# ulysses4ever/SparseMatrixVBCs.jl

Measured on AMD Instinct MI355X. Metric: 1DVBC SpMV effective GB/s (and GFLOP/s) vs HBM roofline, 1/2/4/8 GPU, higher is better.
Workload: dtype f64; 1 GPU; FE-2D-5pt-dof2-10Mx10M-1e8nnz-w2 (SuiteSparse-like mesh operator); op=mul!(y, B', x) -- transposed 1DVBC (multiply_1DVBC.jl:85-180), m=9999392, n=9999392, stripes=4999696, row_blocks=49979072, nnz=99958144, W=8, index_bytes=4, nrhs=1, launch=hipGraph of K products, layout_bytes=826106369, cache=matrix > MALL: every product streams the layout from HBM, parallelism=single GPU

## Files before the change

include/vbc.h:

```cpp
#ifndef VBC_H
#define VBC_H

#ifndef VBC_API
#define VBC_API __attribute__((visibility("default")))
#endif

#include <stddef.h>
#include <stdint.h>

#define VBC_VERSION 30200
#define VBC_INFO_SIZE 152

#ifdef __cplusplus
extern "C" {
#endif

typedef enum vbc_status {
    VBC_OK = 0,
    VBC_DIM_MISMATCH = 1,
    VBC_INVALID_ARG = 2,
    VBC_HIP_ERROR = 3,
    VBC_RCCL_ERROR = 4,
    VBC_UNSUPPORTED_DTYPE = 5,
    VBC_ASSERTION = 6
} vbc_status;

// ... 105 lines not shown
    int32_t device;
    int32_t bins_t, bins_f;
    int64_t device_bytes;
    int64_t bytes_t;
    int64_t bytes_f;
    int32_t bins_m;
    int32_t slot_bins;
    int64_t bytes_m;
    int32_t sweep_bins;
    int32_t planar_bins;
    int32_t planar_run;
    int32_t planar_split;
    int32_t planar_pair;
    int32_t fwd_run;
    int32_t planar_mask;
} vbc_info;

VBC_API int vbc_get_info(const vbc_handle *h, vbc_info *info);

VBC_API int vbc_last_error(char *buf, size_t n);

VBC_API int vbc_version(void);

#ifdef __cplusplus
}
#endif
#endif
```

include/vbc_host.h:

```cpp
#ifndef VBC_HOST_H
#define VBC_HOST_H

#ifndef VBC_API
#define VBC_API __attribute__((visibility("default")))
#endif

#include <stdint.h>

#ifdef __cplusplus
extern "C" {
#endif

VBC_API int vbcx_partition_equi(int64_t n, int64_t w, int64_t *spl, int64_t *L);

VBC_API int vbcx_partition_strict(int64_t m, int64_t n, const int64_t *colptr, const int64_t *rowval,
                          int64_t W, int64_t *spl, int64_t *L);

VBC_API int vbcx_partition_overlap(int64_t m, int64_t n, const int64_t *colptr, const int64_t *rowval,
                           double rho, int64_t W, int64_t *spl, int64_t *L);

VBC_API int vbcx_partition_dynamic(int64_t m, int64_t n, const int64_t *colptr, const int64_t *rowval,
                           int64_t W, double c_stripe, double c_col, double c_pin, double c_row,
                           double c_cell, int64_t *spl, int64_t *L);

// ... 9 lines not shown
                     const int64_t *spl, int64_t *pos, int64_t *ofs);
VBC_API int vbcx_1dvbc_fill(int64_t m, int64_t n, int64_t W, const int64_t *colptr, const int64_t *rowval,
                    const void *nzval, int dtype, int64_t L, const int64_t *spl, const int64_t *pos,
                    const int64_t *ofs, int64_t *idx, void *val, int64_t pad);

VBC_API int vbcx_vbc_count(int64_t m, int64_t n, const int64_t *colptr, const int64_t *rowval, int64_t K,
                   const int64_t *pspl, int64_t L, const int64_t *spl, int64_t *pos, int64_t *ofs);
VBC_API int vbcx_vbc_fill(int64_t m, int64_t n, int64_t U, int64_t W, const int64_t *colptr,
                  const int64_t *rowval, const void *nzval, int dtype, int64_t K,
                  const int64_t *pspl, int64_t L, const int64_t *spl, const int64_t *pos,
                  const int64_t *ofs, int64_t *idx, void *val, int64_t pad);

VBC_API int vbcx_transpose_pattern(int64_t m, int64_t n, const int64_t *colptr, const int64_t *rowval,
                           int64_t *rowptr, int64_t *colval);

#ifdef __cplusplus
}
#endif
#endif
```

sparsematrixvbcs.jl_amd/_lib.py:

```python
import ctypes as C
import os
from pathlib import Path

import numpy as np

PKG_DIR = Path(__file__).resolve().parent
LIB_PATH = Path(os.environ.get("VBC_LIBRARY", PKG_DIR / "libvbc.so"))

VBC_OK, VBC_DIM_MISMATCH, VBC_INVALID_ARG, VBC_HIP_ERROR, VBC_RCCL_ERROR, VBC_UNSUPPORTED_DTYPE, \
    VBC_ASSERTION = range(7)
VBC_F64, VBC_F32, VBC_I64, VBC_I32, VBC_BOOL = range(5)
VBC_MEM_DEVICE, VBC_MEM_HOST = 0, 1
VBC_CREATE_TRANSPOSED, VBC_CREATE_FORWARD, VBC_CREATE_MULTI, VBC_CREATE_SERIAL = 0x1, 0x2, 0x4, 0x8
VBC_CREATE_MULTI_FORWARD = 0x10
VBC_VERSION_MAJOR = 3
VBC_INFO_SIZE = 152
VBC_MUL_REFERENCE_QUIRKS = 0x1
VBC_MAT_ROWMAJOR = 0x2
VBC_SPLIT_STRIPES, VBC_SPLIT_ROWS, VBC_SPLIT_AUTO = 0, 1, 2

ABI_SYMBOLS = (
    "vbc1d_create", "vbc2d_create", "vbc_csc_create", "vbc_destroy", "vbc_mul", "vbc_mul_mat",
    "vbc1d_create_ex", "vbc2d_create_ex", "vbc_csc_create_ex", "vbc_mul_ex", "vbc_mul_mat_ex",
    "vbc_get_info", "vbc_last_error", "vbc_version",
    "vbc1d_create_sharded", "vbc2d_create_sharded", "vbc_sharded_mul", "vbc_sharded_mul_ex", "vbc_sharded_destroy",
    "vbc_sharded_count", "vbc_sharded_shard", "vbc_sharded_split", "vbc_sharded_xspan",
    "vbcx_partition_equi", "vbcx_partition_strict", "vbcx_partition_overlap",
    "vbcx_partition_dynamic", "vbcx_partition_dynamic_table", "vbcx_partition_block", "vbcx_1dvbc_count", "vbcx_1dvbc_fill", "vbcx_vbc_count",
    "vbcx_vbc_fill", "vbcx_transpose_pattern",
)


class DimensionMismatch(ValueError):
    """Julia's DimensionMismatch (multiply_1DVBC.jl:44-45,139-140)."""


class ArgumentError(ValueError):
    """Julia's ArgumentError (SparseMatrixVBCs.jl:45-50,72-79)."""


class HIPError(RuntimeError):
    pass


# ... 4 lines not shown
class vbc_types(C.Structure):
    _fields_ = [("val_dtype", C.c_int32), ("index_bits", C.c_int32), ("compute_dtype", C.c_int32),
                ("reserved", C.c_int32)]


class vbc_info(C.Structure):
    _fields_ = [("m", C.c_int64), ("n", C.c_int64), ("L", C.c_int64), ("K", C.c_int64),
                ("nblocks", C.c_int64), ("nrows", C.c_int64), ("nval", C.c_int64),
                ("nnz_hint", C.c_int64), ("dtype", C.c_int32), ("device", C.c_int32),
                ("bins_t", C.c_int32), ("bins_f", C.c_int32), ("device_bytes", C.c_int64),
                ("bytes_t", C.c_int64), ("bytes_f", C.c_int64), ("bins_m", C.c_int32),
                ("slot_bins", C.c_int32), ("bytes_m", C.c_int64),
                ("sweep_bins", C.c_int32), ("planar_bins", C.c_int32),
                ("planar_run", C.c_int32), ("planar_split", C.c_int32),
                ("planar_pair", C.c_int32), ("fwd_run", C.c_int32),
                ("planar_mask", C.c_int32)]


_lib = None


def lib():
    global _lib
    if _lib is None:
        if not LIB_PATH.exists():
            raise ImportError(f"libvbc.so not found at {LIB_PATH}; build it with `make -C {PKG_DIR}` "
                              "or __graft_entry__.build()")
        try:
            import torch
        except ImportError:
            pass
# ... 27 lines not shown
        L.vbc_mul_mat.argtypes = [P, INT, I64, P, I64, I64, P, I64, I64, D, D, INT, P, U]
        L.vbc_mul_mat_ex.argtypes = [P, INT, I64, P, INT, I64, I64, P, INT, I64, I64, D, D, INT, P, U]
        L.vbc_get_info.argtypes = [P, C.POINTER(vbc_info)]
        L.vbc_last_error.argtypes = [C.c_char_p, C.c_size_t]
        L.vbcx_partition_equi.argtypes = [I64, I64, P, P]
        L.vbcx_partition_strict.argtypes = [I64, I64, P, P, I64, P, P]
        L.vbcx_partition_overlap.argtypes = [I64, I64, P, P, D, I64, P, P]
        L.vbcx_partition_dynamic.argtypes = [I64, I64, P, P, I64, D, D, D, D, D, P, P]
        L.vbcx_partition_dynamic_table.argtypes = [I64, I64, P, P, I64, P, P, P, P]
        L.vbcx_partition_block.argtypes = [I64, I64, P, P, P, I64, I64, P, I64, P, P, P, P]
        L.vbcx_1dvbc_count.argtypes = [I64, I64, P, P, I64, P, P, P]
        L.vbcx_1dvbc_fill.argtypes = [I64, I64, I64, P, P, P, INT, I64, P, P, P, P, P, I64]
        L.vbcx_vbc_count.argtypes = [I64, I64, P, P, I64, P, I64, P, P, P]
        L.vbcx_vbc_fill.argtypes = [I64, I64, I64, I64, P, P, P, INT, I64, P, I64, P, P, P, P, P, I64]
        L.vbcx_transpose_pattern.argtypes = [I64, I64, P, P, P, P]
        _lib = L
    return _lib


def last_error():
    buf = C.create_string_buffer(1024)
    lib().vbc_last_error(buf, 1024)
    return buf.value.decode(errors="replace")


def check(status, what=""):
    if status == VBC_OK:
        return
    msg = f"{what}: {last_error()}" if what else last_error()
    if status == VBC_DIM_MISMATCH:
# ... 37 lines not shown
```

sparsematrixvbcs.jl_amd/csrc/vbc_device.hip:

```cpp
#include <hip/hip_runtime.h>

#include <algorithm>
#include <array>
#include <cstdarg>
#include <cstring>
#include <cmath>
#include <map>
#include <string>
#include <type_traits>
#include <unordered_map>
#include <vector>

#include "vbc_handle.h"
#include "vbc_planar.h"

namespace vbc {

static thread_local std::string g_err;

void set_error(const char *fmt, ...)
{
    char buf[1024];
    va_list ap;
    va_start(ap, fmt);
// ... 407 lines not shown
    int64_t nr = (int64_t)std::llround(share);
    const double quantum = share / std::max(1, planar ? h->occ_p : h->occ_s[kind]);
    if (!planar && h->range_bytes > 0 && share >= 2 * quantum) {
        const double bytes = (double)rows * RPI * (w * esz + 4);
        if (bytes / share < (double)h->range_bytes) nr = (int64_t)std::llround(share / 2);
    }
    const int wps = (pair && h->planar_wps_pair > 0) ? h->planar_wps_pair : h->planar_wps;
    if (planar && split == 1 && wps > 0) nr = std::min<int64_t>(nr, std::max<int64_t>(1, std::llround(quantum * wps)));
    nr = std::max<int64_t>(1, std::min<int64_t>(nr, nch));
    const int64_t qi = (int64_t)quantum;
    if (split == 1 && qi >= 1 && nr < (int64_t)std::llround(share) && nr > qi) nr = nr / qi * qi;
    if (split > 1) nr = nch;
    bool affine = true;
    for (size_t q = 1; q < out.size() && affine; q++)
        affine = (int64_t)out[q] == (int64_t)out[0] + (int64_t)q * (out[1] - out[0]);
    std::vector<int32_t> rrow{0}, rchunk{0};
    int64_t acc = 0;
    for (int64_t c = 0; c < nch; c++) {
        acc += cr[c];
        const bool full = split > 1 || (!affine && (int64_t)(c + 2 - rchunk.back()) * RPI > kSlotOutEntries);
        if (c + 1 < nch && (full || ((int64_t)rrow.size() < nr && acc * nr >= (int64_t)rrow.size() * rows))) {
            rrow.push_back((int32_t)acc);
            rchunk.push_back((int32_t)(c + 1));
        }
    }
    rrow.push_back((int32_t)rows);
    nr = (int64_t)rchunk.size();
    if (layout_knob("VBC_VERBOSE"))
        fprintf(stderr, "[vbc] slot bin kind %d w %d planar %d pair %d run %d split %d chunks %lld rows %lld ranges %lld "
                "(target share %.0f)\n", kind, w, (int)planar, (int)pair, run, split, (long long)nch, (long long)rows,
                (long long)nr, share);
    ps = PendingSlot{};
    SlotBin &b = ps.b;
    b.kind = kind;
    b.wkey = w <= 8 ? w : 0;
    b.w = w;
    b.wst = wsrc;
    b.rpi = RPI;
    b.range0 = range0;
    b.nranges = (int32_t)nr;
    b.nseg = (int32_t)nstripes;
    b.ks = ks;
    b.fused = (planar && kind == 0 && split > 1 && h->small_split > 1 && wsrc <= 8 && ((h->fuse_w >> wsrc) & 1)) ? 1 : 0;
    b.u = h->slot_u;
    b.diag = h->diag;
    b.xcd = (planar && split == 1) ? h->xcd_p : 0;
    b.nowonly = h->slot_wonly ? 0 : 1;
    b.spl = slot_spl(h, kind, w);
    b.planar = planar ? 1 : 0;
    b.run = run;
    b.split = split;
    b.pair = pair ? 1 : 0;
    b.mask = (mask && planar && split == 1 && (!pair || h->planar_mask_pair)) ? 1 : 0;
    b.holes = holes ? 1 : 0;
    if (holes && (split == 1 || pair)) return fail(VBC_INVALID_ARG, "internal: runs with holes need the split product");
    if (planar && split > 1) {
        const double rows_per_wave = (double)rows / (double)std::max<int64_t>(nch, 1) / split;
        const int u0 = (9 / w) / run * run;
        const double step_rows = (double)std::min(8 * run, std::max(run, u0));
        b.deep = h->split_pipe >= 0 ? h->split_pipe : (b.fused && rows_per_wave > h->split_deep * step_rows ? 2 : 0);
        if (b.deep == 2 && h->split_nt_bytes > 0 && (double)h->nval * h->esz > (double)h->split_nt_bytes) b.deep = 3;
    }
    b.out_affine = 1;
    b.out_base = out.empty() ? 0 : out[0];
    b.out_stride = out.size() > 1 ? out[1] - out[0] : 0;
    for (size_t q = 1; q < out.size() && b.out_affine; q++)
        b.out_affine = (int64_t)out[q] == (int64_t)out[0] + (int64_t)q * b.out_stride;
    if (ablation_knob("VBC_NO_AFFINE")) b.out_affine = 0;
// ... 49 lines not shown
                        key[e] = kPad | last;
                    }
                    blk[4 * sl + 0] = v[0][0];
                    blk[4 * sl + 1] = v[0][1];
                    blk[4 * sl + 2] = v[0][2];
                    blk[4 * sl + 3] = v[1][2];
                    blk[128 + 2 * sl + 0] = v[1][0];
                    blk[128 + 2 * sl + 1] = v[1][1];
                    blk[192 + sl] = v[2][2];
                    blk[224 + 2 * sl + 0] = v[2][0];
                    blk[224 + 2 * sl + 1] = v[2][1];
                }
            }
        }
    }
    for (int64_t c = 0; c < (pair ? 0 : nch); c++) {
        for (int32_t qr = 0; qr < cr[c]; qr++, row++) {
            const uint32_t last = qr + run == cr[c] ? kLast : 0u;
            if (b.mask) {
                uint32_t nl = 0;
                for (int sl = 0; sl < RPI; sl++) {
                    const int64_t seg = c * RPI + sl;
                    if (seg < nseg && sbeg[seg] + qr < sbeg[seg + 1]) {
                        if (nl != (uint32_t)sl) return fail(VBC_INVALID_ARG, "masked planar chunk: live lanes not a prefix");
                        nl++;
                    }
                }
                ar.at<uint32_t>(ps.o_nlive)[row] = nl;
            }
            for (int sl = 0; sl < RPI; sl++) {
                const int64_t seg = c * RPI + sl, e = row * RPI + sl;
// ... 1994 lines not shown
    if (const char *e = layout_knob("VBC_SLOTS_PAD")) h->slots_pad = atof(e);
    if (const char *e = layout_knob("VBC_SLOTS_SORT")) h->slots_sort = atoi(e);
    if (const char *e = tuning_knob("VBC_SLOT_NARROW")) h->slot_narrow = atoi(e) != 0;
    if (const char *e = layout_knob("VBC_XCD")) h->xcd = atoi(e) != 0;
    if (const char *e = layout_knob("VBC_XCD_P")) h->xcd_p = atoi(e) != 0;
    if (const char *e = layout_knob("VBC_SLOT_KEYS16")) h->slot_keys16 = atoi(e);
    if (const char *e = layout_knob("VBC_SLOT_DEDUP")) h->slot_dedup = atoi(e) != 0;
    if (const char *e = layout_knob("VBC_SWEEP")) h->sweep_mode = atoi(e) == 0 ? 0 : atoi(e) == 1 ? 1 : -1;
    h->sweep_tile = (h->esz == 8 ? 4 : 2) * kSweepTileBytes;
    h->sweep_pack = h->esz == 8;
    if (const char *e = layout_knob("VBC_FORK")) h->fork = atoi(e) != 0;
    if (const char *e = tuning_knob("VBC_FORK_SIDE_KB")) h->fork_side_bytes = atof(e) * 1024.0;
    if (const char *e = layout_knob("VBC_SWEEP_PACK")) h->sweep_pack = atoi(e) != 0;
    if (const char *e = layout_knob("VBC_SWEEP_TILE")) h->sweep_tile = atoi(e) >= 32 ? 4 * kSweepTileBytes : atoi(e) >= 16 ? 2 * kSweepTileBytes : kSweepTileBytes;
    if (const char *e = layout_knob("VBC_SLOT_STAGE")) h->slot_stage = (atoi(e) == 4 || atoi(e) == 8) ? atoi(e) : 0;
    if (const char *e = layout_knob("VBC_SLOT_PLANAR")) h->slot_planar = atoi(e) == 0 ? 0 : atoi(e) == 1 ? 1 : -1;
    if (const char *e = layout_knob("VBC_SLOT_RUNS")) h->slot_runs = atoi(e) != 0;
    if (const char *e = layout_knob("VBC_PLANAR_PAIR")) h->planar_pair = atoi(e) == 0 ? 0 : atoi(e) == 2 ? 2 : 1;
    if (const char *e = layout_knob("VBC_PLANAR_MASK")) h->planar_mask = atoi(e) != 0;
    if (const char *e = layout_knob("VBC_PLANAR_MASK_PAIR")) h->planar_mask_pair = atoi(e) != 0;
    if (const char *e = layout_knob("VBC_MASK_WINDOW")) h->mask_window = std::max(1, std::min(64, atoi(e)));
    if (const char *e = layout_knob("VBC_PLANAR_SPLIT")) {
        const int v = atoi(e);
        h->planar_split = v == 0 ? 0 : (v == 2 || v == 4 || v == 8) ? v : -1;
    }
    if (flags & VBC_CREATE_SERIAL) {
        h->planar_split = 0;
        if (h->slots_mode < 0) h->slots_mode = 1;
    }
    h->occ_p = std::max(1, std::min(occupancy_planar(h->esz), 8));
    h->target_ranges_l = prop.multiProcessorCount * std::max(1, std::min(occupancy_lanes(h->esz), 8)) * kWavesPerBlock;
    if (const char *e = layout_knob("VBC_PLANAR_LANES")) h->planar_lanes = atoi(e) == 0 ? 0 : atoi(e) == 1 ? 1 : -1;
    if (const char *e = layout_knob("VBC_TARGET_RANGES_L")) h->target_ranges_l = std::max(1, atoi(e));
    if (const char *e = tuning_knob("VBC_LANES_DEEP")) h->lanes_deep = atoi(e) != 0;
    if (const char *e = tuning_knob("VBC_LANES_RDIV")) h->lanes_rdiv = std::max(1, atoi(e));
    if (const char *e = layout_knob("VBC_LANES_PAIR")) h->lanes_pair = atoi(e) != 0;
    if (const char *e = tuning_knob("VBC_SPLIT_KC")) h->split_kc = atoi(e) != 0;
    if (const char *e = tuning_knob("VBC_SPLIT_ROWS")) h->split_rows = std::max(1, atoi(e));
    if (const char *e = layout_knob("VBC_SMALL_FUSE")) h->small_fuse = atoi(e);
    if (const char *e = layout_knob("VBC_SIDE_FUSE")) h->side_fuse = atoi(e) < 0 ? -1 : atoi(e) != 0;
    if (const char *e = layout_knob("VBC_COLSPLIT")) h->colsplit = atoi(e) != 0;
    if (const char *e = tuning_knob("VBC_FUSE_PMAX")) h->fuse_pmax = atoi(e) >= 8 ? 8 : atoi(e) >= 4 ? 4 : 2;
    if (const char *e = tuning_knob("VBC_COLSPLIT_W")) h->colsplit_w = std::max(0, atoi(e));
// ... 381 lines not shown
        for (const SlotBin &b : h->lt.pbins)
            if (b.ks > 1) info->planar_mask |= 64;
    info->fwd_run = 1;
    if (h->has_f)
        for (const auto &l : h->lf)
            for (const auto &b : l.pbins) {
                info->fwd_run = std::max<int32_t>(info->fwd_run, b.lanes ? b.wkey : b.run);
                if (b.mask && !b.lanes) info->planar_mask |= 2;
                if (b.split > 1) info->planar_mask |= 8;
                if (b.lanes) info->planar_mask |= 16;
                if (b.dot) info->planar_mask |= 2048;
            }
    if (h->has_ft)
        for (const SlotBin &b : h->lft.pbins)
            if (b.split > 1) info->planar_mask |= 8;
    info->bytes_m = h->has_m ? h->bytes_m : h->bytes_mf;
    return VBC_OK;
}

static int check_mul(const vbc_handle *h, int trans, int64_t nx, int64_t ny, bool mat = false)
{
    if (!h) return fail(VBC_INVALID_ARG, "NULL handle");
    const int64_t want_x = trans ? h->m : h->n, want_y = trans ? h->n : h->m;
    if (nx != want_x || ny != want_y) return fail(VBC_DIM_MISMATCH, "DimensionMismatch");
    if (trans && !h->has_t && !(mat && h->has_m))
        return fail(VBC_INVALID_ARG, mat ? "handle built without VBC_CREATE_TRANSPOSED or VBC_CREATE_MULTI"
                                         : "handle built without VBC_CREATE_TRANSPOSED");
    if (!trans && !h->has_f && !(mat && h->has_mf))
        return fail(VBC_INVALID_ARG, mat ? "handle built without VBC_CREATE_FORWARD or VBC_CREATE_MULTI_FORWARD"
                                         : "handle built without VBC_CREATE_FORWARD");
// ... 357 lines not shown
```

sparsematrixvbcs.jl_amd/csrc/vbc_handle.h:

```cpp
#pragma once
#include <hip/hip_runtime.h>

#include <cstdint>
#include <mutex>
#include <vector>

#include "vbc_internal.h"
#include "vbc_kernels.h"
#include "vbc_panel.h"
#include "vbc_tiles.h"

namespace vbc {

#define VBC_HIP(call)                                                                             \
    do {                                                                                          \
        hipError_t e_ = (call);                                                                   \
        if (e_ != hipSuccess) {                                                                   \
            set_error("%s failed: %s", #call, hipGetErrorString(e_));                             \
            return VBC_HIP_ERROR;                                                                 \
        }                                                                                         \
    } while (0)

struct Launch {
    std::vector<Bin> bins;
// ... 95 lines not shown
    int slots_mode = -1;
    double slots_pad = 1.10;
    int slot_narrow = 1;
    int slots_sort = 1;
    int xcd = 1;
    int64_t range_bytes = 192 << 10;
    int xcd_p = 1;
    int occ_s[2] = {4, 4};
    int64_t slot_rows_padded = 0, slot_rows_real = 0;
    int64_t slot_rows_padded_last = 0;
    int slot_u = 0;
    bool slot_dedup = true;
    int slot_keys16 = 1;
    int fork = 1;
    int slot_stage = -1;
    int slot_planar = -1;
    int slot_runs = 1;
    int planar_pair = 1;
    int planar_mask = 1;
    int planar_mask_pair = 1;
    int mask_window = 2;
    int planar_split = -1;
    int target_ranges_p = 4096;
    int target_ranges_l = 4096;
    int slot_wonly = 1;
    int split_kc = 0;
    int small_split = 0;
    uint32_t fuse_w = 0;
    int small_fuse = 1;
    int side_fuse = -1;
// ... 54 lines not shown
```

sparsematrixvbcs.jl_amd/csrc/vbc_host.cpp:

```cpp
#include <algorithm>
#include <cmath>
#include <cstdlib>
#include <cstring>
#include <limits>
#include <thread>
#include <vector>

#include "vbc_host.h"
#include "vbc_internal.h"

using vbc::fail;

namespace {

int host_threads()
{
    if (const char *e = std::getenv("VBC_HOST_THREADS")) return std::max(1, std::atoi(e));
    const unsigned hc = std::thread::hardware_concurrency();
    return (int)std::max(1u, std::min(hc ? hc : 1u, 16u));
}

template <typename F>
int parallel_ranges(int64_t n, int64_t work, F f)
{
// ... 417 lines not shown
int vbcx_transpose_pattern(int64_t m, int64_t n, const int64_t *colptr, const int64_t *rowval,
                           int64_t *rowptr, int64_t *colval)
{
    if (int st = check_csc(m, n, colptr, rowval)) return st;
    std::fill(rowptr, rowptr + m + 1, 0);
    for (int64_t p = 0; p < colptr[n] - 1; p++) rowptr[rowval[p]]++;
    rowptr[0] = 1;
    for (int64_t i = 0; i < m; i++) rowptr[i + 1] += rowptr[i];
    std::vector<int64_t> next(rowptr, rowptr + m);
    for (int64_t j = 0; j < n; j++)
        for (int64_t p = colptr[j] - 1; p < colptr[j + 1] - 1; p++)
            colval[(next[rowval[p] - 1]++) - 1] = j + 1;
    return VBC_OK;
}

}
```

sparsematrixvbcs.jl_amd/csrc/vbc_internal.h:

```cpp
#pragma once
#include <cstdarg>
#include <cstdint>
#include <cstdio>
#include <cstdlib>

#include "vbc.h"

namespace vbc {

void set_error(const char *fmt, ...) __attribute__((format(printf, 1, 2)));

inline int fail(int status, const char *what)
{
    set_error("%s", what);
    return status;
}

inline const char *layout_knob(const char *name) { return std::getenv(name); }
#ifdef VBC_ABLATION
#define VBC_ABL(expr) (expr)
inline const char *ablation_knob(const char *name) { return std::getenv(name); }
inline const char *tuning_knob(const char *name) { return std::getenv(name); }
#else
#define VBC_ABL(expr) 0
inline const char *ablation_knob(const char *) { return nullptr; }
inline const char *tuning_knob(const char *) { return nullptr; }
#endif

inline int elem_size(int dtype)
{
    switch (dtype) {
    case VBC_F64: case VBC_I64: return 8;
    case VBC_F32: case VBC_I32: return 4;
    case VBC_BOOL: return 1;
    default: return 0;
    }
}

template <typename To>
void host_convert(const void *src, int dt, int64_t n, int64_t inc, To *dst)
{
    const char *p = static_cast<const char *>(src);
// ... 35 lines not shown
```

sparsematrixvbcs.jl_amd/csrc/vbc_kernels.h:

```cpp
#pragma once
#include <hip/hip_runtime.h>

#include <cstdint>

#include "vbc_internal.h"

namespace vbc {

constexpr int kBlockThreads = 256;
constexpr int kWavesPerBlock = kBlockThreads / 64;
constexpr int kTileKDefault = 8;
constexpr int kPipeDefault = 2;
constexpr uint32_t kHead = 0x80000000u;

template <typename T>
using gptr = __attribute__((address_space(1))) T *;
template <typename T>
__device__ __forceinline__ gptr<T> G(T *p) { return (gptr<T>)p; }
template <typename T>
__device__ __forceinline__ gptr<const T> G(const T *p) { return (gptr<const T>)p; }

template <typename V>
__device__ __forceinline__ void st_y(gptr<V> p, V v, bool nt)
{
// ... 58 lines not shown
    const uint32_t *base;
    const uint32_t *kdoff;
    const void *val;
    const int32_t *out;
    const int32_t *rrow;
    const int32_t *rchunk;
    const uint32_t *nlive;
    int32_t lanes;
    int32_t ntiles;
    int32_t deep;
    int32_t nowonly;
    const int32_t *trow;
    const int32_t *tseg;
    const int16_t *lseg;
    int32_t dot;
    int32_t pad_dot;
};

constexpr uint32_t kHoleIdx = (1u << 27) - 1;
constexpr int kHoleShift = 27;

constexpr int kSplitParts = 16;
struct SplitPart {
    int32_t w, run, chunk0, nseg, out_affine, out_base, out_stride, wst, holes, ks;
    const int32_t *rrow;
    const uint32_t *key;
    const void *val;
    const int32_t *out;
};
struct SplitMulti {
    int32_t nparts, nchunks, pad0, pad1;
// ... 779 lines not shown
```

sparsematrixvbcs.jl_amd/csrc/vbc_slots.h:

```cpp
#pragma once
#include "vbc_kernels.h"

namespace vbc {

template <typename T, int V>
__device__ __forceinline__ T slot_reduce(const T (&v)[V], int lane, int sub, int LPR)
{
    T s = T(0);
#pragma unroll
    for (int e = 0; e < V; e++) s += v[e];
    for (int d = 1; d < LPR; d <<= 1) {
        const T t = __shfl(s, (lane + d) & 63, 64);
        if (sub + d < LPR) s += t;
    }
    return s;
}

template <typename T, int KIND, int W_, int U, bool FASTE, int DIAG = 0, int NB = 0, bool KC = false>
__device__ __forceinline__ void run_slots(const SlotBin &b, int r, int lane, const T *__restrict__ x,
                                          T *__restrict__ y, T alpha, T beta, bool rd, char *lds_wave, int *lds_out)
{
    constexpr bool kGeneric = (W_ == 0);
    constexpr int V = kGeneric ? 1 : vec_elems(sizeof(T), W_);
    const int w = kGeneric ? b.w : W_;
    const int LPR = kGeneric ? b.w : W_ / V;
    const int RPI = b.rpi;
    const int slot = lane / LPR, sub = lane - slot * LPR;
    const bool active = slot < RPI;
    const int R0 = G(b.rrow)[r], R1 = G(b.rrow)[r + 1];
    if (R0 >= R1) return;
    int c = G(b.rchunk)[r];
    const int lslot = active ? slot : 0, lsub = active ? sub : 0;
    const gptr<const T> val = G(static_cast<const T *>(b.val));
    const gptr<const uint32_t> key = G(b.key);
    const gptr<const T> xg = G(x);
    constexpr int XV = KIND == 0 ? 1 : V;

    typedef __attribute__((address_space(4))) const uint32_t *cptr;
    const cptr bases = (cptr)b.base;
    const cptr doffs = (cptr)b.kdoff;
    auto load = [&](int R, uint32_t (&kk)[U], uint32_t (&bs)[U], T (&v)[U][V]) {
#pragma unroll
        for (int u = 0; u < U; u++) {
            const int Rc = min(R + u, R1 - 1);
            const size_t p = (size_t)Rc * RPI + lslot;
            if constexpr (KC) {
// ... 7 lines not shown
        }
    };
    constexpr uint32_t kPad16 = 0xFFFF8000u;
    auto gather = [&](const uint32_t (&kk)[U], const uint32_t (&bs)[U], T (&xv)[U][XV]) {
#pragma unroll
        for (int u = 0; u < U; u++) {
            const uint32_t gi = KC ? (bs[u] & kSlotIdx) + (kk[u] == kPad16 ? 0u : kk[u]) : kk[u] & kSlotIdx;
#pragma unroll
            for (int e = 0; e < XV; e++) xv[u][e] = DIAG == 2 ? T(1) : xg[gi + (KIND == 0 ? 0 : lsub * V + e)];
        }
    };
    T acc[V], dump[V];
#pragma unroll
    for (int e = 0; e < V; e++) acc[e] = dump[e] = T(0);
    int nbuf = 0, cfirst = c;
    const int c0 = c;
    if constexpr (!FASTE) {
        if (!b.out_affine) {
            const int n = min(kSlotOutEntries, b.nseg - c0 * RPI);
            for (int i = lane; i < n; i += 64) lds_out[i] = G(b.out)[c0 * RPI + i];
        }
    }

    auto write_out = [&]() {
        const int64_t segs = min((int64_t)nbuf * RPI, (int64_t)b.nseg - (int64_t)cfirst * RPI);
        const int64_t bytes = segs * (KIND == 0 ? w : 1) * (int64_t)sizeof(T);
        char *dst = reinterpret_cast<char *>(y + b.out_base + (int64_t)cfirst * RPI * b.out_stride);
        if ((reinterpret_cast<uintptr_t>(dst) & 15) == 0) {
            typedef uint32_t u4 __attribute__((ext_vector_type(4)));
            for (int64_t off = (int64_t)lane * 16; off < bytes; off += 1024) {
// ... 17 lines not shown
        if constexpr (NB > 0) {
            if constexpr (KIND == 0) {
                typedef T vt __attribute__((ext_vector_type(V)));
                vt t;
#pragma unroll
                for (int e = 0; e < V; e++) t[e] = alpha * acc[e];
                *reinterpret_cast<vt *>(lds_wave + ((size_t)nbuf * 64 + lane) * V * sizeof(T)) = t;
            } else {
                const T s = slot_reduce<T, V>(acc, lane, sub, LPR);
                if (sub == 0 && active) reinterpret_cast<T *>(lds_wave)[(size_t)nbuf * RPI + slot] = alpha * s;
            }
#pragma unroll
            for (int e = 0; e < V; e++) acc[e] = T(0);
            if (nbuf == 0) cfirst = c;
            c++;
            if (++nbuf == NB) write_out();
            return;
        }
        if constexpr (KIND == 0) {
            if (ok) {
                const int o = (FASTE || b.out_affine) ? b.out_base + seg * b.out_stride : lds_out[(c - c0) * RPI + slot];
                gptr<T> yo = DIAG == 4 ? G(y) + ((size_t)r * 64 + lane) * V : G(y) + o + sub * V;
                const int lim = b.wst - sub * V;
                T q[V];
#pragma unroll
                for (int e = 0; e < V; e++) {
                    q[e] = alpha * acc[e];
                    if (!FASTE && rd && e < lim) q[e] = fmadd(beta, yo[e], q[e]);
                }
                if constexpr (DIAG == 1) {
#pragma unroll
// ... 12 lines not shown
                }
            }
        } else {
            const T s = slot_reduce<T, V>(acc, lane, sub, LPR);
            if (ok && sub == 0) {
                const int o = (FASTE || b.out_affine) ? b.out_base + seg * b.out_stride : lds_out[(c - c0) * RPI + slot];
                gptr<T> yo = G(y) + o;
                T q = alpha * s;
                if (!FASTE && rd) q = fmadd(beta, *yo, q);
                *yo = q;
            }
        }
#pragma unroll
        for (int e = 0; e < V; e++) acc[e] = T(0);
        c++;
    };
    int R1v;
    asm volatile("v_mov_b32 %0, %1" : "=v"(R1v) : "s"(R1));
    auto compute = [&](int R, const uint32_t (&kk)[U], const uint32_t (&bs)[U], const T (&v)[U][V],
                       const T (&xv)[U][XV]) {
#pragma unroll
        for (int u = 0; u < U; u++) {
            const bool live = R + u < R1v;
            const bool pad = KC ? kk[u] == kPad16 : (kk[u] & kPad) != 0;
#pragma unroll
            for (int e = 0; e < V; e++) {
                const T xe = pad ? T(0) : xv[u][KIND == 0 ? 0 : e];
                const T nv = fmadd(v[u][e], xe, acc[e]);
                acc[e] = live ? nv : acc[e];
            }
// ... 21 lines not shown
#pragma unroll
        for (int e = 0; e < V; e++) G(y)[(size_t)(blockIdx.x * kBlockThreads + threadIdx.x) * V + e] = dump[e];
    }
}

template <typename T, int W_, int SPL, int U, bool FASTE, int NB, bool KC>
__device__ __forceinline__ void run_slots_narrow(const SlotBin &b, int r, int lane, const T *__restrict__ x,
                                                 T *__restrict__ y, T alpha, T beta, bool rd, char *lds_wave,
                                                 int *lds_out)
{
    constexpr int NV = SPL * W_;
    const int RPI = b.rpi;
    const int R0 = G(b.rrow)[r], R1 = G(b.rrow)[r + 1];
    if (R0 >= R1) return;
    int c = G(b.rchunk)[r];
    const gptr<const T> val = G(static_cast<const T *>(b.val));
    const gptr<const T> xg = G(x);
    typedef __attribute__((address_space(4))) const uint32_t *cptr;
    const cptr bases = (cptr)b.base;
    const cptr doffs = (cptr)b.kdoff;
    typedef T vt __attribute__((ext_vector_type(NV)));
    auto load = [&](int R, uint32_t (&kk)[U][SPL], uint32_t (&bs)[U], T (&v)[U][NV]) {
#pragma unroll
        for (int u = 0; u < U; u++) {
            const int Rc = min(R + u, R1 - 1);
            const size_t p = (size_t)Rc * RPI + (size_t)lane * SPL;
            if constexpr (KC) {
                typedef int16_t hv __attribute__((ext_vector_type(SPL)));
                const hv d = *(gptr<const hv>)((gptr<const int16_t>)b.key + (size_t)doffs[Rc] + (size_t)lane * SPL);
#pragma unroll
// ... 13 lines not shown
    };
    constexpr uint32_t kPad16 = 0xFFFF8000u;
    auto is_pad = [&](uint32_t k) { return KC ? k == kPad16 : (k & kPad) != 0; };
    auto gather = [&](const uint32_t (&kk)[U][SPL], const uint32_t (&bs)[U], T (&xv)[U][SPL]) {
#pragma unroll
        for (int u = 0; u < U; u++)
#pragma unroll
            for (int k = 0; k < SPL; k++) {
                const uint32_t gi = KC ? (bs[u] & kSlotIdx) + (kk[u][k] == kPad16 ? 0u : kk[u][k]) : kk[u][k] & kSlotIdx;
                xv[u][k] = xg[gi];
            }
    };
    T acc[NV];
#pragma unroll
    for (int e = 0; e < NV; e++) acc[e] = T(0);
    int nbuf = 0, cfirst = c;
    const int c0 = c;
    if constexpr (!FASTE) {
        if (!b.out_affine) {
            const int n = min(kSlotOutEntries, b.nseg - c0 * RPI);
            for (int i = lane; i < n; i += 64) lds_out[i] = G(b.out)[c0 * RPI + i];
        }
    }
    auto write_out = [&]() {
        const int64_t segs = min((int64_t)nbuf * RPI, (int64_t)b.nseg - (int64_t)cfirst * RPI);
        const int64_t bytes = segs * W_ * (int64_t)sizeof(T);
        char *dst = reinterpret_cast<char *>(y + b.out_base + (int64_t)cfirst * RPI * b.out_stride);
        if ((reinterpret_cast<uintptr_t>(dst) & 15) == 0) {
            typedef uint32_t u4 __attribute__((ext_vector_type(4)));
            for (int64_t off = (int64_t)lane * 16; off < bytes; off += 1024) {
                if (off + 16 <= bytes) {
// ... 34 lines not shown
#pragma unroll
                        for (int e = 0; e < W_; e++) {
                            if (e >= lim) break;
                            T q = alpha * acc[k * W_ + e];
                            if (!FASTE && rd) q = fmadd(beta, G(y)[o + e], q);
                            G(y)[o + e] = q;
                        }
                    }
                }
            }
        }
#pragma unroll
        for (int e = 0; e < NV; e++) acc[e] = T(0);
        c++;
        if constexpr (NB > 0) {
            if (++nbuf == NB) write_out();
        }
    };
    int R1v;
    asm volatile("v_mov_b32 %0, %1" : "=v"(R1v) : "s"(R1));
    auto compute = [&](int R, const uint32_t (&kk)[U][SPL], const uint32_t (&bs)[U], const T (&v)[U][NV],
                       const T (&xv)[U][SPL]) {
#pragma unroll
        for (int u = 0; u < U; u++) {
            const bool live = R + u < R1v;
#pragma unroll
            for (int k = 0; k < SPL; k++) {
                const T xe = is_pad(kk[u][k]) ? T(0) : xv[u][k];
#pragma unroll
                for (int e = 0; e < W_; e++) {
                    const T nv = fmadd(v[u][k * W_ + e], xe, acc[k * W_ + e]);
// ... 81 lines not shown
```

Measured before the change: 7245 GB/s.

## Interleave slot-bin chunk ranges into sweeping pieces to align x gather locality

Adds a host planner that samples column-offset deltas in transposed slot bins and, when a few dominant far offsets exist, reorders chunks so each wave range processes strided pieces of P chunks and all ranges sweep the matrix together. Concurrent waves then touch nearby x regions, which is meant to improve cache reuse of the x gather. The kernels gain a piece counter that jumps chunk indices after each burst. It also adds equal-sized range counting by default and exposes the plan in the info struct. The risks are more irregular output write bursts and a heuristic that may pick poor plans or none at all.

```diff
diff --git a/include/vbc.h b/include/vbc.h
--- a/include/vbc.h
+++ b/include/vbc.h
@@ -8,8 +8,8 @@
 #include <stddef.h>
 #include <stdint.h>
 
-#define VBC_VERSION 30200
-#define VBC_INFO_SIZE 152
+#define VBC_VERSION 30300
+#define VBC_INFO_SIZE 160
 
 #ifdef __cplusplus
 extern "C" {
@@ -145,6 +145,9 @@
     int32_t planar_pair;
     int32_t fwd_run;
     int32_t planar_mask;
+    int32_t slot_sweep_p;
+    int32_t slot_sweep_s;
+    int32_t slot_sweep_r;
 } vbc_info;
 
 VBC_API int vbc_get_info(const vbc_handle *h, vbc_info *info);
diff --git a/include/vbc_host.h b/include/vbc_host.h
--- a/include/vbc_host.h
+++ b/include/vbc_host.h
@@ -47,6 +47,9 @@
 VBC_API int vbcx_transpose_pattern(int64_t m, int64_t n, const int64_t *colptr, const int64_t *rowval,
                            int64_t *rowptr, int64_t *colval);
 
+VBC_API int vbcx_slot_sweep_plan(int64_t chunks, int64_t slots, int nb, int ndelta, const double *delta,
+                                 const double *weight, int force_p, int force_s, int64_t *plan);
+
 #ifdef __cplusplus
 }
 #endif
diff --git a/sparsematrixvbcs.jl_amd/_lib.py b/sparsematrixvbcs.jl_amd/_lib.py
--- a/sparsematrixvbcs.jl_amd/_lib.py
+++ b/sparsematrixvbcs.jl_amd/_lib.py
@@ -14,7 +14,7 @@
 VBC_CREATE_TRANSPOSED, VBC_CREATE_FORWARD, VBC_CREATE_MULTI, VBC_CREATE_SERIAL = 0x1, 0x2, 0x4, 0x8
 VBC_CREATE_MULTI_FORWARD = 0x10
 VBC_VERSION_MAJOR = 3
-VBC_INFO_SIZE = 152
+VBC_INFO_SIZE = 160
 VBC_MUL_REFERENCE_QUIRKS = 0x1
 VBC_MAT_ROWMAJOR = 0x2
 VBC_SPLIT_STRIPES, VBC_SPLIT_ROWS, VBC_SPLIT_AUTO = 0, 1, 2
@@ -27,7 +27,7 @@
     "vbc_sharded_count", "vbc_sharded_shard", "vbc_sharded_split", "vbc_sharded_xspan",
     "vbcx_partition_equi", "vbcx_partition_strict", "vbcx_partition_overlap",
     "vbcx_partition_dynamic", "vbcx_partition_dynamic_table", "vbcx_partition_block", "vbcx_1dvbc_count", "vbcx_1dvbc_fill", "vbcx_vbc_count",
-    "vbcx_vbc_fill", "vbcx_transpose_pattern",
+    "vbcx_vbc_fill", "vbcx_transpose_pattern", "vbcx_slot_sweep_plan",
 )
 
 
@@ -62,7 +62,8 @@
                 ("sweep_bins", C.c_int32), ("planar_bins", C.c_int32),
                 ("planar_run", C.c_int32), ("planar_split", C.c_int32),
                 ("planar_pair", C.c_int32), ("fwd_run", C.c_int32),
-                ("planar_mask", C.c_int32)]
+                ("planar_mask", C.c_int32), ("slot_sweep_p", C.c_int32),
+                ("slot_sweep_s", C.c_int32), ("slot_sweep_r", C.c_int32)]
 
 
 _lib = None
@@ -120,6 +121,7 @@
         L.vbcx_vbc_count.argtypes = [I64, I64, P, P, I64, P, I64, P, P, P]
         L.vbcx_vbc_fill.argtypes = [I64, I64, I64, I64, P, P, P, INT, I64, P, I64, P, P, P, P, P, I64]
         L.vbcx_transpose_pattern.argtypes = [I64, I64, P, P, P, P]
+        L.vbcx_slot_sweep_plan.argtypes = [I64, I64, INT, INT, P, P, INT, INT, P]
         _lib = L
     return _lib
 
diff --git a/sparsematrixvbcs.jl_amd/csrc/vbc_device.hip b/sparsematrixvbcs.jl_amd/csrc/vbc_device.hip
--- a/sparsematrixvbcs.jl_amd/csrc/vbc_device.hip
+++ b/sparsematrixvbcs.jl_amd/csrc/vbc_device.hip
@@ -445,9 +445,67 @@
     bool affine = true;
     for (size_t q = 1; q < out.size() && affine; q++)
         affine = (int64_t)out[q] == (int64_t)out[0] + (int64_t)q * (out[1] - out[0]);
+    SweepPlan sweep;
+    {
+        const int V0 = w <= 8 ? vec_elems(esz, w) : 1;
+        const bool full0 = slot_spl(h, kind, w) > 1 || (RPI * (w / V0) == 64 && V0 * esz <= 16);
+        const int64_t ostride = out.size() > 1 ? (int64_t)out[1] - out[0] : 0;
+        const bool eligible = h->slot_sweep != 0 && kind == 0 && !planar && split == 1 && ks == 1 && order.empty() &&
+                              !mask && affine && !ablation_knob("VBC_NO_AFFINE") && full0 && wsrc == w &&
+                              (nseg <= 1 || ostride == w) && nch >= 2;
+        if (eligible && h->slot_sweep == 2) {
+            sweep = plan_slot_sweep(nch, nr, 8, 0, nullptr, nullptr, h->slot_sweep_p, h->slot_sweep_s);
+        } else if (eligible && nch >= nr) {
+            std::unordered_map<int64_t, int64_t> hist;
+            std::vector<int64_t> all;
+            const int64_t step = std::max<int64_t>(1, nseg / 65536);
+            for (int64_t q = 0; q < nseg; q += step)
+                for (int64_t t = sbeg[q]; t < sbeg[q + 1]; t++) {
+                    const int64_t d = (int64_t)(ents[pstart[q] + (t - sbeg[q])].key & kSlotIdx) - (int64_t)out[q];
+                    all.push_back(d >= 0 ? d / w : -((-d + w - 1) / w));
+                }
+            if (!all.empty()) {
+                std::nth_element(all.begin(), all.begin() + all.size() / 2, all.end());
+                const int64_t med = all[all.size() / 2];
+                int64_t far = 0;
+                for (int64_t d : all)
+                    if (std::llabs(d - med) > (int64_t)8 * RPI) {
+                        hist[d - med]++;
+                        far++;
+                    }
+                std::vector<double> dl, wt;
+                int64_t dom = 0;
+                for (const auto &kv : hist)
+                    if (kv.second * 10 >= far) {
+                        dl.push_back((double)kv.first / RPI);
+                        wt.push_back((double)kv.second);
+                        dom += kv.second;
+                    }
+                if (far * 20 >= (int64_t)all.size() && dom * 5 >= far * 4)
+                    sweep = plan_slot_sweep(nch, nr, 8, (int)dl.size(), dl.data(), wt.data(), 0, 0);
+            }
+        }
+    }
+    if (sweep.P == 0 && h->slot_equal && !planar && split == 1 && affine && nch > nr) nr = equal_range_count(nch, nr);
+    std::vector<int64_t> lorder;
     std::vector<int32_t> rrow{0}, rchunk{0};
     int64_t acc = 0;
-    for (int64_t c = 0; c < nch; c++) {
+    if (sweep.P > 0) {
+        const int64_t P = sweep.P, pieces = (nch + P - 1) / P;
+        lorder.reserve(nch);
+        for (int64_t r = 0; r < sweep.R; r++) {
+            for (int64_t p = r; p < pieces; p += sweep.R)
+                for (int64_t c = p * P; c < std::min(nch, (p + 1) * P); c++) {
+                    lorder.push_back(c);
+                    acc += cr[c];
+                }
+            if (r + 1 < sweep.R) {
+                rrow.push_back((int32_t)acc);
+                rchunk.push_back((int32_t)((r + 1) * P));
+            }
+        }
+    }
+    for (int64_t c = 0; c < (sweep.P > 0 ? 0 : nch); c++) {
         acc += cr[c];
         const bool full = split > 1 || (!affine && (int64_t)(c + 2 - rchunk.back()) * RPI > kSlotOutEntries);
         if (c + 1 < nch && (full || ((int64_t)rrow.size() < nr && acc * nr >= (int64_t)rrow.size() * rows))) {
@@ -459,8 +517,8 @@
     nr = (int64_t)rchunk.size();
     if (layout_knob("VBC_VERBOSE"))
         fprintf(stderr, "[vbc] slot bin kind %d w %d planar %d pair %d run %d split %d chunks %lld rows %lld ranges %lld "
-                "(target share %.0f)\n", kind, w, (int)planar, (int)pair, run, split, (long long)nch, (long long)rows,
-                (long long)nr, share);
+                "(target share %.0f) pieces of %d chunks, %lld sweeps (lag %.3f)\n", kind, w, (int)planar, (int)pair, run,
+                split, (long long)nch, (long long)rows, (long long)nr, share, (int)sweep.P, (long long)sweep.S, sweep.lag);
     ps = PendingSlot{};
     SlotBin &b = ps.b;
     b.kind = kind;
@@ -483,6 +541,7 @@
     b.split = split;
     b.pair = pair ? 1 : 0;
     b.mask = (mask && planar && split == 1 && (!pair || h->planar_mask_pair)) ? 1 : 0;
+    b.piece = sweep.P;
     b.holes = holes ? 1 : 0;
     if (holes && (split == 1 || pair)) return fail(VBC_INVALID_ARG, "internal: runs with holes need the split product");
     if (planar && split > 1) {
@@ -562,7 +621,8 @@
             }
         }
     }
-    for (int64_t c = 0; c < (pair ? 0 : nch); c++) {
+    for (int64_t lc = 0; lc < (pair ? 0 : nch); lc++) {
+        const int64_t c = lorder.empty() ? lc : lorder[lc];
         for (int32_t qr = 0; qr < cr[c]; qr++, row++) {
             const uint32_t last = qr + run == cr[c] ? kLast : 0u;
             if (b.mask) {
@@ -2587,6 +2647,17 @@
     if (const char *e = layout_knob("VBC_SWEEP_PACK")) h->sweep_pack = atoi(e) != 0;
     if (const char *e = layout_knob("VBC_SWEEP_TILE")) h->sweep_tile = atoi(e) >= 32 ? 4 * kSweepTileBytes : atoi(e) >= 16 ? 2 * kSweepTileBytes : kSweepTileBytes;
     if (const char *e = layout_knob("VBC_SLOT_STAGE")) h->slot_stage = (atoi(e) == 4 || atoi(e) == 8) ? atoi(e) : 0;
+    if (const char *e = layout_knob("VBC_SLOT_SWEEP")) {
+        if (e[0] == 'p' || e[0] == 'P') {
+            h->slot_sweep = 2;
+            h->slot_sweep_p = std::max(1, atoi(e + 1));
+            const char *sl = std::strchr(e, '/');
+            h->slot_sweep_s = sl ? std::max(0, atoi(sl + 1)) : 0;
+        } else {
+            h->slot_sweep = atoi(e) != 0;
+        }
+    }
+    if (const char *e = layout_knob("VBC_SLOT_EQUAL")) h->slot_equal = atoi(e) != 0;
     if (const char *e = layout_knob("VBC_SLOT_PLANAR")) h->slot_planar = atoi(e) == 0 ? 0 : atoi(e) == 1 ? 1 : -1;
     if (const char *e = layout_knob("VBC_SLOT_RUNS")) h->slot_runs = atoi(e) != 0;
     if (const char *e = layout_knob("VBC_PLANAR_PAIR")) h->planar_pair = atoi(e) == 0 ? 0 : atoi(e) == 2 ? 2 : 1;
@@ -2600,6 +2671,7 @@
     if (flags & VBC_CREATE_SERIAL) {
         h->planar_split = 0;
         if (h->slots_mode < 0) h->slots_mode = 1;
+        h->slot_sweep = 0;
     }
     h->occ_p = std::max(1, std::min(occupancy_planar(h->esz), 8));
     h->target_ranges_l = prop.multiProcessorCount * std::max(1, std::min(occupancy_lanes(h->esz), 8)) * kWavesPerBlock;
@@ -3011,6 +3083,16 @@
     if (h->has_ft)
         for (const SlotBin &b : h->lft.pbins)
             if (b.split > 1) info->planar_mask |= 8;
+    if (h->has_t)
+        for (const SlotBin &b : h->lt.sbins) {
+            if (b.kind != 0 || (info->slot_sweep_r > 0 && b.piece == 0)) continue;
+            info->slot_sweep_r = b.nranges;
+            if (b.piece == 0) continue;
+            const int64_t nch = ((int64_t)b.nseg + b.rpi - 1) / b.rpi, pieces = (nch + b.piece - 1) / b.piece;
+            info->slot_sweep_p = b.piece;
+            info->slot_sweep_s = (int32_t)((pieces + b.nranges - 1) / b.nranges);
+            break;
+        }
     info->bytes_m = h->has_m ? h->bytes_m : h->bytes_mf;
     return VBC_OK;
 }
diff --git a/sparsematrixvbcs.jl_amd/csrc/vbc_handle.h b/sparsematrixvbcs.jl_amd/csrc/vbc_handle.h
--- a/sparsematrixvbcs.jl_amd/csrc/vbc_handle.h
+++ b/sparsematrixvbcs.jl_amd/csrc/vbc_handle.h
@@ -133,6 +133,9 @@
     int slot_keys16 = 1;
     int fork = 1;
     int slot_stage = -1;
+    int slot_sweep = 1;
+    int slot_sweep_p = 0, slot_sweep_s = 0;
+    int slot_equal = 1;
     int slot_planar = -1;
     int slot_runs = 1;
     int planar_pair = 1;
diff --git a/sparsematrixvbcs.jl_amd/csrc/vbc_host.cpp b/sparsematrixvbcs.jl_amd/csrc/vbc_host.cpp
--- a/sparsematrixvbcs.jl_amd/csrc/vbc_host.cpp
+++ b/sparsematrixvbcs.jl_amd/csrc/vbc_host.cpp
@@ -455,4 +455,69 @@
     return VBC_OK;
 }
 
-}
+int vbcx_slot_sweep_plan(int64_t chunks, int64_t slots, int nb, int ndelta, const double *delta,
+                         const double *weight, int force_p, int force_s, int64_t *plan)
+{
+    if (chunks < 0 || slots < 1 || nb < 1 || ndelta < 0 || !plan || (ndelta > 0 && (!delta || !weight)))
+        return fail(VBC_INVALID_ARG, "vbcx_slot_sweep_plan: bad arguments");
+    const vbc::SweepPlan sp = vbc::plan_slot_sweep(chunks, slots, nb, ndelta, delta, weight, force_p, force_s);
+    plan[0] = sp.P;
+    plan[1] = sp.S;
+    plan[2] = sp.P > 0 ? sp.R : vbc::equal_range_count(chunks, slots);
+    return VBC_OK;
+}
+
+}
+
+namespace vbc {
+
+SweepPlan plan_slot_sweep(int64_t chunks, int64_t slots, int nb, int ndelta, const double *delta,
+                          const double *weight, int force_p, int force_s)
+{
+    SweepPlan best;
+    if (chunks < 1 || slots < 1) return best;
+    auto shape = [&](int P, int64_t sweeps, SweepPlan &sp) {
+        const int64_t pieces = (chunks + P - 1) / P;
+        int64_t S = sweeps > 0 ? std::min(sweeps, pieces) : (pieces + slots - 1) / slots;
+        sp.P = P;
+        sp.R = (pieces + S - 1) / S;
+        sp.S = (pieces + sp.R - 1) / sp.R;
+        return pieces;
+    };
+    if (force_p > 0) {
+        shape(std::min(force_p, nb), force_s, best);
+        return best;
+    }
+    double wsum = 0;
+    for (int i = 0; i < ndelta; i++) wsum += weight[i];
+    if (ndelta == 0 || wsum <= 0) return best;
+    int64_t best_lagq = 0, best_len = 0;
+    for (int P = 1; P <= nb; P++) {
+        SweepPlan sp;
+        const int64_t pieces = shape(P, 0, sp);
+        if (pieces < slots || (double)sp.R < 0.9 * (double)slots) continue;
+        for (int i = 0; i < ndelta; i++) {
+            const double q = std::fabs(delta[i]) / P;
+            sp.lag += weight[i] * std::fabs(q - std::round(q)) * P;
+        }
+        sp.lag /= wsum;
+        const int64_t lagq = std::llround(sp.lag * 4), len = sp.S * P;
+        if (best.P == 0 || lagq < best_lagq || (lagq == best_lagq && len <= best_len)) {
+            best = sp;
+            best_lagq = lagq;
+            best_len = len;
+        }
+    }
+    if (best.P > 0 && best.lag >= 0.45) best = SweepPlan{};
+    return best;
+}
+
+int64_t equal_range_count(int64_t chunks, int64_t slots)
+{
+    if (chunks <= slots) return std::max<int64_t>(chunks, 1);
+    const int64_t k = (chunks + slots - 1) / slots;
+    const int64_t fill = (int64_t)std::ceil(0.9 * (double)slots);
+    return std::min(slots, std::max((chunks + k - 1) / k, fill));
+}
+
+}
diff --git a/sparsematrixvbcs.jl_amd/csrc/vbc_internal.h b/sparsematrixvbcs.jl_amd/csrc/vbc_internal.h
--- a/sparsematrixvbcs.jl_amd/csrc/vbc_internal.h
+++ b/sparsematrixvbcs.jl_amd/csrc/vbc_internal.h
@@ -26,6 +26,15 @@
 inline const char *ablation_knob(const char *) { return nullptr; }
 inline const char *tuning_knob(const char *) { return nullptr; }
 #endif
+
+struct SweepPlan {
+    int32_t P = 0;
+    int64_t S = 0, R = 0;
+    double lag = 0;
+};
+SweepPlan plan_slot_sweep(int64_t chunks, int64_t slots, int nb, int ndelta, const double *delta,
+                          const double *weight, int force_p, int force_s);
+int64_t equal_range_count(int64_t chunks, int64_t slots);
 
 inline int elem_size(int dtype)
 {
diff --git a/sparsematrixvbcs.jl_amd/csrc/vbc_kernels.h b/sparsematrixvbcs.jl_amd/csrc/vbc_kernels.h
--- a/sparsematrixvbcs.jl_amd/csrc/vbc_kernels.h
+++ b/sparsematrixvbcs.jl_amd/csrc/vbc_kernels.h
@@ -96,7 +96,7 @@
     const int32_t *tseg;
     const int16_t *lseg;
     int32_t dot;
-    int32_t pad_dot;
+    int32_t piece;
 };
 
 constexpr uint32_t kHoleIdx = (1u << 27) - 1;
diff --git a/sparsematrixvbcs.jl_amd/csrc/vbc_slots.h b/sparsematrixvbcs.jl_amd/csrc/vbc_slots.h
--- a/sparsematrixvbcs.jl_amd/csrc/vbc_slots.h
+++ b/sparsematrixvbcs.jl_amd/csrc/vbc_slots.h
@@ -30,6 +30,8 @@
     const int R0 = G(b.rrow)[r], R1 = G(b.rrow)[r + 1];
     if (R0 >= R1) return;
     int c = G(b.rchunk)[r];
+    const int burst = (NB > 0 && b.piece > 0) ? b.piece : NB;
+    const int pjump = b.piece > 0 ? (b.nranges - 1) * b.piece : 0;
     const int lslot = active ? slot : 0, lsub = active ? sub : 0;
     const gptr<const T> val = G(static_cast<const T *>(b.val));
     const gptr<const uint32_t> key = G(b.key);
@@ -67,6 +69,7 @@
 #pragma unroll
     for (int e = 0; e < V; e++) acc[e] = dump[e] = T(0);
     int nbuf = 0, cfirst = c;
+    int pk = 0;
     const int c0 = c;
     if constexpr (!FASTE) {
         if (!b.out_affine) {
@@ -114,7 +117,10 @@
             for (int e = 0; e < V; e++) acc[e] = T(0);
             if (nbuf == 0) cfirst = c;
             c++;
-            if (++nbuf == NB) write_out();
+            if (++nbuf == burst) {
+                write_out();
+                c += pjump;
+            }
             return;
         }
         if constexpr (KIND == 0) {
@@ -157,6 +163,10 @@
 #pragma unroll
         for (int e = 0; e < V; e++) acc[e] = T(0);
         c++;
+        if (b.piece > 0 && ++pk == b.piece) {
+            pk = 0;
+            c += pjump;
+        }
     };
     int R1v;
     asm volatile("v_mov_b32 %0, %1" : "=v"(R1v) : "s"(R1));
@@ -208,6 +218,8 @@
     const int R0 = G(b.rrow)[r], R1 = G(b.rrow)[r + 1];
     if (R0 >= R1) return;
     int c = G(b.rchunk)[r];
+    const int burst = (NB > 0 && b.piece > 0) ? b.piece : NB;
+    const int pjump = b.piece > 0 ? (b.nranges - 1) * b.piece : 0;
     const gptr<const T> val = G(static_cast<const T *>(b.val));
     const gptr<const T> xg = G(x);
     typedef __attribute__((address_space(4))) const uint32_t *cptr;
@@ -251,7 +263,7 @@
     T acc[NV];
 #pragma unroll
     for (int e = 0; e < NV; e++) acc[e] = T(0);
-    int nbuf = 0, cfirst = c;
+    int nbuf = 0, cfirst = c, pk = 0;
     const int c0 = c;
     if constexpr (!FASTE) {
         if (!b.out_affine) {
@@ -316,7 +328,13 @@
         for (int e = 0; e < NV; e++) acc[e] = T(0);
         c++;
         if constexpr (NB > 0) {
-            if (++nbuf == NB) write_out();
+            if (++nbuf == burst) {
+                write_out();
+                c += pjump;
+            }
+        } else if (b.piece > 0 && ++pk == b.piece) {
+            pk = 0;
+            c += pjump;
         }
     };
     int R1v;
```

Measured after the change: 6963 GB/s. 3.9% lower.
